# ralexstokes/ethereum_consensus

Measured on NVIDIA H100. Metric: fast_aggregate_verify tuples/s, higher is better.
Workload: dtype u32 limbs (381-bit Fp), u32 SHA-256 words

## Files before the change

ethereum_consensus_b200/csrc/groups.cuh:

```cuda
#pragma once
#include "curve.cuh"
#include "fpl.cuh"

namespace b200 {

enum : int32_t {
    BLS_SUCCESS = 0, BLS_BAD_ENCODING = 1, BLS_POINT_NOT_ON_CURVE = 2, BLS_POINT_NOT_IN_GROUP = 3,
    BLS_AGGR_TYPE_MISMATCH = 4, BLS_VERIFY_FAIL = 5, BLS_PK_IS_INFINITY = 6, BLS_BAD_SCALAR = 7
};

typedef Aff<Fp> G1Aff;
typedef Jac<Fp> G1Jac;
typedef Aff<Fp2> G2Aff;
typedef Jac<Fp2> G2Jac;

B200_HD bool fp_from_be48_masked(Fp& r, const uint8_t* b, bool mask_flags) {
    Fp raw;
    fp_from_be_bytes_raw(raw, b);
    if (mask_flags) raw.l[11] &= 0x1fffffffu;
    const Fp p = fp_p();
    if (fp_geq_raw(raw, p)) return false;
    fp_to_mont(r, raw);
    return true;
}
B200_HD bool bytes_all_zero(const uint8_t* b, int n) {
    uint32_t acc = 0;
    for (int i = 0; i < n; i++) acc |= b[i];
    return acc == 0;
}

B200_HD int32_t g1_uncompress(G1Aff& out, const uint8_t b[48]) {
    const uint8_t f = b[0];
    out.inf = 0;
    if (!(f & 0x80)) return BLS_BAD_ENCODING;
    if (f & 0x40) {
        if ((f & 0x3f) == 0 && bytes_all_zero(b + 1, 47)) { out.inf = 1; out.x = fp_zero(); out.y = fp_zero(); return BLS_SUCCESS; }
        return BLS_BAD_ENCODING;
    }
    Fp x, y2, y;
    if (!fp_from_be48_masked(x, b, true)) return BLS_BAD_ENCODING;
    fp_sqr(y2, x);
    fp_mul(y2, y2, x);
    const Fp four = B200_FP_B_G1;
    fp_add(y2, y2, four);
    if (!fp_sqrt(y, y2)) return BLS_POINT_NOT_ON_CURVE;
    if (fp_is_lex_largest(y) != ((f & 0x20) != 0)) fp_neg(y, y);
    out.x = x; out.y = y;
    return BLS_SUCCESS;
}

B200_HD bool g1_in_subgroup(const G1Aff& p) {
    if (p.inf) return true;
    G1Jac t, t2;
    jac_mul_u64(t, p.x, p.y, B200_Z_ABS);
    jac_mul_u64_jac(t2, t, B200_Z_ABS);
    const Fp beta = B200_FP_BETA;
    Fp bx, ny;
    fp_mul(bx, p.x, beta);
    fp_neg(ny, p.y);
    return jac_eq_aff(t2, bx, ny);
}

B200_HD int32_t g1_uncompress_lazy(G1Aff& out, const uint8_t b[48]) {
    const uint8_t f = b[0];
    out.inf = 0;
    if (!(f & 0x80)) return BLS_BAD_ENCODING;
    if (f & 0x40) {
        if ((f & 0x3f) == 0 && bytes_all_zero(b + 1, 47)) { out.inf = 1; out.x = fp_zero(); out.y = fp_zero(); return BLS_SUCCESS; }
        return BLS_BAD_ENCODING;
    }
    Fp x;
    if (!fp_from_be48_masked(x, b, true)) return BLS_BAD_ENCODING;
    FpL xl = fpl_from_fp(x), y2, yl, c;
    f_sqr(y2, xl);
    f_mul(y2, y2, xl);
    f_add(y2, y2, curve_b<FpL>());
    fpl_pow(yl, y2, B200_EXP_TABLE(exp_sqrt));
    f_sqr(c, yl);
    if (!f_eq(c, y2)) return BLS_POINT_NOT_ON_CURVE;
    Fp y = fpl_canon(yl);
    if (fp_is_lex_largest(y) != ((f & 0x20) != 0)) fp_neg(y, y);
    out.x = x; out.y = y;
    return BLS_SUCCESS;
}
B200_HD bool g1_in_subgroup_lazy(const G1Aff& p) {
    if (p.inf) return true;
    const FpL px = fpl_from_fp(p.x), py = fpl_from_fp(p.y);
    Jac<FpL> t, t2;
    jac_mul_u64(t, px, py, B200_Z_ABS);
    jac_mul_u64_jac(t2, t, B200_Z_ABS);
    const Fp beta = B200_FP_BETA;
    FpL bx, ny;
    f_mul(bx, px, fpl_from_fp(beta));
    f_neg(ny, py);
    return jac_eq_aff(t2, bx, ny);
}

B200_HD int32_t g1_key_validate(G1Aff& out, const uint8_t b[48]) {
#if defined(B200_G1_CANONICAL_FP)
    int32_t rc = g1_uncompress(out, b);
    if (rc) return rc;
    if (out.inf) return BLS_PK_IS_INFINITY;
    if (!g1_in_subgroup(out)) return BLS_POINT_NOT_IN_GROUP;
#else
    int32_t rc = g1_uncompress_lazy(out, b);
    if (rc) return rc;
    if (out.inf) return BLS_PK_IS_INFINITY;
    if (!g1_in_subgroup_lazy(out)) return BLS_POINT_NOT_IN_GROUP;
#endif
    return BLS_SUCCESS;
}

B200_HD void g1_compress(uint8_t out[48], const G1Aff& a) {
    if (a.inf) { for (int i = 0; i < 48; i++) out[i] = 0; out[0] = 0xc0; return; }
    Fp raw;
    fp_from_mont(raw, a.x);
    fp_to_be_bytes_raw(out, raw);
    out[0] |= 0x80;
    if (fp_is_lex_largest(a.y)) out[0] |= 0x20;
}

B200_BIG int32_t g2_uncompress(G2Aff& out, const uint8_t b[96]) {
    const uint8_t f = b[0];
    out.inf = 0;
    if (!(f & 0x80)) return BLS_BAD_ENCODING;
    if (f & 0x40) {
        if ((f & 0x3f) == 0 && bytes_all_zero(b + 1, 95)) { out.inf = 1; out.x = fp2_zero(); out.y = fp2_zero(); return BLS_SUCCESS; }
        return BLS_BAD_ENCODING;
    }
    Fp2 x, y2, y;
    if (!fp_from_be48_masked(x.c1, b, true)) return BLS_BAD_ENCODING;
    if (!fp_from_be48_masked(x.c0, b + 48, false)) return BLS_BAD_ENCODING;
    fp2_sqr(y2, x);
    fp2_mul(y2, y2, x);
    const Fp2 bb = B200_FP2_B_G2;
    fp2_add(y2, y2, bb);
    if (!fp2_sqrt(y, y2)) return BLS_POINT_NOT_ON_CURVE;
    if (fp2_is_lex_largest(y) != ((f & 0x20) != 0)) fp2_neg(y, y);
    out.x = x; out.y = y;
    return BLS_SUCCESS;
}

B200_HD void g2_compress(uint8_t out[96], const G2Aff& a) {
    if (a.inf) { for (int i = 0; i < 96; i++) out[i] = 0; out[0] = 0xc0; return; }
    Fp raw;
    fp_from_mont(raw, a.x.c1);
    fp_to_be_bytes_raw(out, raw);
    fp_from_mont(raw, a.x.c0);
// ... 52 lines not shown
```

ethereum_consensus_b200/build.py:

```python
from __future__ import annotations

import os
import subprocess
import sys
from concurrent.futures import ThreadPoolExecutor
from pathlib import Path

PKG = Path(__file__).resolve().parent
CSRC = PKG / "csrc"
LIB = PKG / "libb200_consensus.so"
OBJ = PKG / "build"
NVCC = os.environ.get("NVCC", "/usr/local/cuda/bin/nvcc")
ARCH = ["-gencode", "arch=compute_90a,code=sm_90a"]
FLAGS = [*ARCH, "-lineinfo", "-O3", "-std=c++17",
         "-Xcompiler", "-fPIC,-fvisibility=hidden", "--expt-relaxed-constexpr"]
DEFAULT_PTXAS_OPT = {"bls_g1.cu": 1, "bls_g2.cu": 1, "bls_vm.cu": 1}


def _stale(target: Path, deps) -> bool:
    if not target.exists():
        return True
    t = target.stat().st_mtime
    return any(Path(d).stat().st_mtime > t for d in deps)


def build(force: bool = False, verbose: bool = False, defines=(), suffix: str = "", ptxas_opt=None) -> Path:
    global LIB, OBJ
    env_opt = {kv.split(":")[0]: int(kv.split(":")[1]) for kv in os.environ.get("B200_PTXAS_OPT", "").split(",") if kv}
    ptxas_opt = {**DEFAULT_PTXAS_OPT, **env_opt, **dict(ptxas_opt or {})}
    if suffix:
        LIB = PKG / f"libb200_consensus{suffix}.so"
        OBJ = PKG / f"build{suffix}"
    srcs = sorted(CSRC.glob("*.cu"))
    hdrs = sorted(CSRC.glob("*.cuh")) + sorted(CSRC.glob("*.h")) + sorted((PKG.parent / "include").glob("*.h"))
    OBJ.mkdir(exist_ok=True)
    jobs = []
    def command(s, o):
        cmd = [NVCC, *FLAGS, *[f"-D{d}" for d in defines], "-c", str(s), "-o", str(o)]
        if s.name in ptxas_opt and int(ptxas_opt[s.name]) != 3:
            cmd[1:1] = ["-Xptxas", f"-O{int(ptxas_opt[s.name])}"]
        return cmd

    for s in srcs:
        o = OBJ / (s.stem + ".o")
        stamp = o.with_suffix(".cmd")
        if force or _stale(o, [s] + hdrs) or not stamp.exists() or stamp.read_text() != " ".join(command(s, o)):
            jobs.append((s, o))

    def cc(job):
        s, o = job
        cmd = command(s, o)
        stamp = o.with_suffix(".cmd")
        if verbose:
            cmd.insert(1, "-Xptxas=-v")
        r = subprocess.run(cmd, capture_output=True, text=True)
        if r.returncode != 0:
            raise RuntimeError(f"nvcc failed for {s.name}:\n{r.stdout}\n{r.stderr}")
        stamp.write_text(" ".join(command(s, o)))
        return r.stderr

    with ThreadPoolExecutor(max_workers=min(8, max(1, len(jobs)))) as ex:
        for msg in ex.map(cc, jobs):
            if verbose and msg:
                print(msg, file=sys.stderr)
    objs = [OBJ / (s.stem + ".o") for s in srcs]
    if force or jobs or _stale(LIB, objs):
        cmd = [NVCC, "-shared", "-o", str(LIB), *map(str, objs), *ARCH,
               "-Xcompiler", "-fPIC", "-cudart", "static"]
        r = subprocess.run(cmd, capture_output=True, text=True)
# ... 12 lines not shown
```

ethereum_consensus_b200/crypto.py:

```python
from __future__ import annotations

import ctypes as C
from typing import Sequence

import numpy as np

from . import _lib
from .ssz import hash

BLS_DST = b"BLS_SIG_BLS12381G2_XMD:SHA-256_SSWU_RO_POP_"
BLS_PUBLIC_KEY_BYTES_LEN = 48
BLS_SIGNATURE_BYTES_LEN = 96
INFINITY_COMPRESSED_SIGNATURE = bytes([0xC0]) + bytes(95)

_BLST_TEXT = {1: "bad encoding", 2: "point not on curve", 3: "point not in group", 4: "aggregation type mismatch",
              5: "verification failed", 6: "public key is infinity", 7: "bad scalar input"}

_lib.register_protos({
    "b200_verify_signature": (C.c_int32, [C.c_void_p, C.c_void_p, C.c_size_t, C.c_void_p]),
    "b200_fast_aggregate_verify": (C.c_int32, [C.c_void_p, C.c_size_t, C.c_void_p, C.c_size_t, C.c_void_p]),
    "b200_eth_fast_aggregate_verify": (C.c_int32, [C.c_void_p, C.c_size_t, C.c_void_p, C.c_size_t, C.c_void_p]),
    "b200_aggregate_verify": (C.c_int32, [C.c_void_p, C.c_size_t, C.c_void_p, C.c_void_p, C.c_size_t, C.c_void_p]),
    "b200_aggregate": (C.c_int32, [C.c_void_p, C.c_size_t, C.c_void_p]),
    "b200_eth_aggregate_public_keys": (C.c_int32, [C.c_void_p, C.c_size_t, C.c_void_p]),
# ... 173 lines not shown

    def __init__(self, pks_flat):
        n = (pks_flat.nbytes if hasattr(pks_flat, "nbytes") else len(pks_flat)) // 48
        _lib.check(_lib.lib().b200_registry_load(_lib.ptr(pks_flat), n), "registry_load")
        self.n = n

    def key_codes(self) -> np.ndarray:
        out = np.empty(max(self.n, 1), dtype=np.int32)
        _lib.check(_lib.lib().b200_registry_key_codes(_lib.ptr(out), self.n), "registry_key_codes")
        return out[:self.n]

    def verify_batch(self, indices, offsets, msgs32, sigs, extra_keys=None) -> np.ndarray:
        idx = np.ascontiguousarray(indices, dtype=np.uint32)
        off = np.ascontiguousarray(offsets, dtype=np.uint32)
        t = _batch_size(off, msgs32, sigs, indices=idx)
        out = np.empty(max(t, 1), dtype=np.int32)
        if extra_keys is not None and _nbytes(extra_keys):
            if _nbytes(extra_keys) % 48:
                raise ValueError("extra keys must be 48 bytes each")
            _lib.check(_lib.lib().b200_fast_aggregate_verify_batch_mixed(_lib.ptr(extra_keys), _nbytes(extra_keys) // 48, _lib.ptr(idx), _lib.ptr(off),
                                                                         _lib.ptr(msgs32), _lib.ptr(sigs), t, _lib.ptr(out)), "verify_batch_mixed")
        else:
            _lib.check(_lib.lib().b200_fast_aggregate_verify_batch_indexed(_lib.ptr(idx), _lib.ptr(off), _lib.ptr(msgs32),
                                                                           _lib.ptr(sigs), t, _lib.ptr(out)), "verify_batch_indexed")
        return out[:t]

    def verify_batch_all(self, indices, offsets, msgs32, sigs, seed: bytes = None) -> bool:
        idx = np.ascontiguousarray(indices, dtype=np.uint32)
        off = np.ascontiguousarray(offsets, dtype=np.uint32)
        t = _batch_size(off, msgs32, sigs, indices=idx, seed=seed)
        sd = np.frombuffer(bytes(seed), dtype=np.uint8) if seed is not None else None
        ok = C.c_int32(0)
        _lib.check(_lib.lib().b200_fast_aggregate_verify_batch_indexed_all(_lib.ptr(idx), _lib.ptr(off), _lib.ptr(msgs32), _lib.ptr(sigs), t,
                                                                           _lib.ptr(sd) if sd is not None else 0, C.byref(ok)), "verify_batch_indexed_all")
        return bool(ok.value)


def last_kernel_ms() -> float:
    return float(_lib.lib().b200_last_kernel_ms())


def last_dominant_kernel_ms() -> float:
    return float(_lib.lib().b200_last_dominant_kernel_ms())


def fp_selftest(n: int = 1 << 16, seed: int = 1) -> int:
    m = C.c_uint32(0)
    _lib.check(_lib.lib().b200_fp_selftest(n, seed, C.byref(m)), "fp_selftest")
    return int(m.value)


FP_EVAL_OPS = {"fp_mul": 0, "fp_sqr": 1, "fpl_mul": 2, "fpl_sqr": 3, "fp_add": 4, "fp_sub": 5, "fp_neg": 6, "fpl_add": 7,
               "fpl_sub": 8, "fpl_neg": 9, "fp_add_raw": 10, "fp_sub_raw": 11, "fp_inv_kaliski": 12, "fp_inv_fermat": 13,
               "fp_sqrt": 14, "fpl_pow_sqrt": 15, "fp_is_lex_largest": 16,
               "fp2_mul": 32, "fp2_sqr": 33, "fp2_inv": 34, "fp2_sqrt": 35, "fp2_sgn0": 36}


def fp_eval(op: str, a, b=None) -> np.ndarray:
    a = np.ascontiguousarray(a, dtype=np.uint32)
    b = np.zeros_like(a) if b is None else np.ascontiguousarray(b, dtype=np.uint32)
    if a.ndim != 2 or a.shape[1] != 24 or b.shape != a.shape:
        raise ValueError("operands must be uint32[n, 24]")
    out = np.zeros((max(a.shape[0], 1), 25), dtype=np.uint32)
    _lib.check(_lib.lib().b200_fp_eval(FP_EVAL_OPS[op], a.shape[0], _lib.ptr(a), _lib.ptr(b), _lib.ptr(out)), f"fp_eval({op})")
    return out[:a.shape[0]]


CURVE_EVAL_OPS = {"g1l_add_mixed": 0, "g1l_add": 1, "g1l_in_subgroup": 2,
                  "g2_add": 32, "g2_add_mixed": 33, "g2_double": 34, "g2_in_subgroup": 35, "g2_psi": 36,
                  "g2_clear_cofactor": 37, "g2_sswu_iso": 38, "g2_h2c_finish": 39}


def curve_eval(op: str, a, b=None) -> np.ndarray:
    a = np.ascontiguousarray(a, dtype=np.uint32)
    b = np.zeros_like(a) if b is None else np.ascontiguousarray(b, dtype=np.uint32)
    if a.ndim != 2 or a.shape[1] != 73 or b.shape != a.shape:
        raise ValueError("operands must be uint32[n, 73]")
    out = np.zeros((max(a.shape[0], 1), 73), dtype=np.uint32)
    _lib.check(_lib.lib().b200_curve_eval(CURVE_EVAL_OPS[op], a.shape[0], _lib.ptr(a), _lib.ptr(b), _lib.ptr(out)),
               f"curve_eval({op})")
    return out[:a.shape[0]]


def tune(knob: str, value: int) -> None:
    _lib.check(_lib.lib().b200_tune(knob.encode(), int(value)), f"tune({knob})")


def vm_load_programs(blob) -> None:
    a = np.ascontiguousarray(blob, dtype=np.uint32)
    _lib.check(_lib.lib().b200_vm_load_programs(_lib.ptr(a), a.size), "vm_load_programs")


def measure_int_peak(kind: int) -> float:
    g = C.c_double(0)
    _lib.check(_lib.lib().b200_measure_int_peak(kind, C.byref(g)), "measure_int_peak")
    return float(g.value)
```

ethereum_consensus_b200/csrc/bls_g1.cu:

```cuda
#if defined(B200_G1_SQR_VIA_MUL)
#define B200_FP_SQR_VIA_MUL 1
#endif
#if !defined(B200_G1_INLINE_MUL)
#define B200_FP_MUL_CALL 1
#endif
#define B200_POW_TAB_SMEM 1
#include <cuda_runtime.h>

#include "bls_kernels.cuh"

namespace b200 {
namespace {

__device__ __forceinline__ void g1_validate_body(const uint8_t* __restrict__ keys, uint32_t n, G1Aff* __restrict__ out,
                                                 int32_t* __restrict__ codes) {
    const uint32_t i = blockIdx.x * blockDim.x + threadIdx.x;
    if (i >= n) return;
    __align__(16) uint8_t b[48];
    const uint4* src = reinterpret_cast<const uint4*>(keys + size_t(i) * 48);
    uint4* dst = reinterpret_cast<uint4*>(b);
    dst[0] = src[0]; dst[1] = src[1]; dst[2] = src[2];
    G1Aff p;
    const int32_t rc = g1_key_validate(p, b);
    codes[i] = rc;
// ... 132 lines not shown
        const uint32_t bu = fp_sub_raw(u, x, y), bv = fp_sub_raw_portable(v, x, y);
        if (bu != bv || !fp_eq(u, v)) bad++;
        fp_add(u, x, y); fp_sub(u, u, y);
        if (!fp_eq(u, x)) bad++;
        fp_sub(u, x, y); fp_sub(v, y, x); fp_neg(v, v);
        if (!fp_eq(u, v)) bad++;
        fp_dbl(u, x); fp_add(v, x, x);
        if (!fp_eq(u, v)) bad++;
        fp_neg(u, x); fp_add(u, u, x);
        if (!fp_is_zero(u)) bad++;
        fp_add_masked_raw(u, x, y, 0u);
        if (!fp_eq(u, x)) bad++;
        fp_add_masked_raw(u, x, y, 0xffffffffu); fp_add_raw_portable(v, x, y);
        if (!fp_eq(u, v)) bad++;
    }
    if ((i & 63) == 0 && !fp_is_zero(a)) {
        fp_inv(t, a); fp_mul(t, t, a);
        if (!fp_eq(t, fp_one())) bad++;
        Fp k, f;
        fp_inv_kaliski(k, a); fp_inv_fermat(f, a);
        if (!fp_eq(k, f)) bad++;
        fp_inv_kaliski(k, fp_zero());
        if (!fp_is_zero(k)) bad++;
    }
    if (bad) atomicAdd(out_mismatch, bad);
}

__global__ void k_fp_eval(int32_t op, uint32_t n, const uint32_t* __restrict__ a, const uint32_t* __restrict__ b,
                          uint32_t* __restrict__ out) {
    const uint32_t i = blockIdx.x * blockDim.x + threadIdx.x;
    if (i >= n) return;
    Fp x, y, r = fp_zero();
    for (int k = 0; k < 12; k++) { x.l[k] = a[size_t(i) * kFpEvalIn + k]; y.l[k] = b[size_t(i) * kFpEvalIn + k]; }
    const FpL xl = fpl_from_fp(x), yl = fpl_from_fp(y);
    FpL rl;
    uint32_t flag = 0;
    switch (op) {
    case FP_EVAL_MUL: fp_mul(r, x, y); break;
    case FP_EVAL_SQR: fp_sqr(r, x); break;
    case FPL_EVAL_MUL: f_mul(rl, xl, yl); r = rl.v; break;
    case FPL_EVAL_SQR: f_sqr(rl, xl); r = rl.v; break;
    case FP_EVAL_ADD: fp_add(r, x, y); break;
    case FP_EVAL_SUB: fp_sub(r, x, y); break;
    case FP_EVAL_NEG: fp_neg(r, x); break;
    case FPL_EVAL_ADD: f_add(rl, xl, yl); r = rl.v; break;
    case FPL_EVAL_SUB: f_sub(rl, xl, yl); r = rl.v; break;
    case FPL_EVAL_NEG: f_neg(rl, xl); r = rl.v; break;
    case FP_EVAL_ADD_RAW: flag = fp_add_raw(r, x, y); break;
    case FP_EVAL_SUB_RAW: flag = fp_sub_raw(r, x, y); break;
    case FP_EVAL_INV_KALISKI: fp_inv_kaliski(r, x); break;
    case FP_EVAL_INV_FERMAT: fp_inv_fermat(r, x); break;
    case FP_EVAL_SQRT: flag = fp_sqrt(r, x) ? 1u : 0u; break;
    case FPL_EVAL_POW_SQRT: fpl_pow(rl, xl, B200_EXP_TABLE(exp_sqrt)); r = rl.v; break;
    case FP_EVAL_IS_LEX_LARGEST: flag = fp_is_lex_largest(x) ? 1u : 0u; break;
    default: break;
    }
    uint32_t* o = out + size_t(i) * kFpEvalOut;
    for (int k = 0; k < 12; k++) { o[k] = r.l[k]; o[12 + k] = 0; }
    o[24] = flag;
}

__global__ void k_curve_eval(int32_t op, uint32_t n, const uint32_t* __restrict__ a, const uint32_t* __restrict__ b,
                             uint32_t* __restrict__ out) {
    const uint32_t i = blockIdx.x * blockDim.x + threadIdx.x;
    if (i >= n) return;
    const uint32_t* pa = a + size_t(i) * kCurveEvalWords;
    const uint32_t* pb = b + size_t(i) * kCurveEvalWords;
    Jac<FpL> p, q, r;
    for (int k = 0; k < 12; k++) {
        p.x.v.l[k] = pa[k]; p.y.v.l[k] = pa[24 + k]; p.z.v.l[k] = pa[48 + k];
        q.x.v.l[k] = pb[k]; q.y.v.l[k] = pb[24 + k]; q.z.v.l[k] = pb[48 + k];
    }
    jac_set_inf(r);
    uint32_t flag = 0;
    switch (op) {
    case CURVE_G1L_ADD_MIXED: jac_add_mixed(r, p, q.x, q.y); break;
    case CURVE_G1L_ADD: jac_add(r, p, q); break;
    case CURVE_G1L_IN_SUBGROUP: {
        G1Aff s;
        s.x = p.x.v; s.y = p.y.v; s.inf = pa[72];
        flag = g1_in_subgroup_lazy(s) ? 1u : 0u;
        break;
    }
    default: break;
    }
    uint32_t* o = out + size_t(i) * kCurveEvalWords;
    for (int k = 0; k < 72; k++) o[k] = 0;
    for (int k = 0; k < 12; k++) { o[k] = r.x.v.l[k]; o[24 + k] = r.y.v.l[k]; o[48 + k] = r.z.v.l[k]; }
    o[72] = flag;
}

}

template <class K>
static size_t with_pow_tab(K kernel, unsigned threads) {
    const size_t bytes = fp_pow_smem_bytes(threads);
    static const void* seen[16];
    static size_t granted[16];
    static int n_seen = 0;
    const void* key = reinterpret_cast<const void*>(kernel);
    for (int i = 0; i < n_seen; i++)
        if (seen[i] == key) {
            if (granted[i] < bytes) { cudaFuncSetAttribute(kernel, cudaFuncAttributeMaxDynamicSharedMemorySize, int(bytes)); granted[i] = bytes; }
            return bytes;
        }
    cudaFuncSetAttribute(kernel, cudaFuncAttributeMaxDynamicSharedMemorySize, int(bytes));
    if (n_seen < 16) { seen[n_seen] = key; granted[n_seen++] = bytes; }
    return bytes;
}
static int g_g1_variant = 7;
static uint32_t g_g1_small_n = 3u * 148u * 384u;
void set_g1_small_n(uint32_t n) { g_g1_small_n = n; }
void set_g1_variant(int v) { if (v >= 0 && v <= 7) g_g1_variant = v; }
void launch_g1_validate(const uint8_t* keys, uint32_t n, G1Aff* out, int32_t* codes, void* stream, int cta) {
    if (!n) return;
    cudaStream_t st = static_cast<cudaStream_t>(stream);
    switch (g_g1_variant) {
    case 6: k_g1_validate_r128<<<(n + 511) / 512, 512, with_pow_tab(k_g1_validate_r128, 512), st>>>(keys, n, out, codes); break;
    case 0: k_g1_validate_main<<<(n + 255) / 256, 256, with_pow_tab(k_g1_validate_main, 256), st>>>(keys, n, out, codes); break;
    default:
        if (cta == 128 || (cta != 384 && n <= g_g1_small_n))
            k_g1_validate_r168<<<(n + 127) / 128, 128, with_pow_tab(k_g1_validate_r168, 128), st>>>(keys, n, out, codes);
        else
            k_g1_validate_r168<<<(n + 383) / 384, 384, with_pow_tab(k_g1_validate_r168, 384), st>>>(keys, n, out, codes);
        break;
    }
}
void launch_g1_aggregate(const G1Aff* keys, const int32_t* key_codes, const uint32_t* index, const uint32_t* off,
                         uint32_t n_tuples, G1Aff* agg, G1Pre* agg_pre, int32_t* pk_code, uint32_t* flags,
                         uint32_t extra_flags, void* stream, G1Jac* agg_jac) {
    if (!n_tuples) return;
    k_g1_aggregate<<<(n_tuples + kAggWarps - 1) / kAggWarps, 32 * kAggWarps, with_pow_tab(k_g1_aggregate, 32 * kAggWarps),
                     static_cast<cudaStream_t>(stream)>>>(
        keys, key_codes, index, off, n_tuples, agg, agg_pre, pk_code, flags, extra_flags, agg_jac);
}
void launch_g1_compress(const G1Aff* p, uint8_t* out48, void* stream) {
    k_g1_compress<<<1, 32, with_pow_tab(k_g1_compress, 32), static_cast<cudaStream_t>(stream)>>>(p, out48);
}
void launch_neg_g1(G1Aff* out, G1Pre* out_pre, void* stream) { k_neg_g1<<<1, 32, 0, static_cast<cudaStream_t>(stream)>>>(out, out_pre); }
void launch_fp_selftest(uint32_t n, uint32_t seed, uint32_t* out_mismatch, void* stream) {
    k_fp_selftest<<<(n + 127) / 128, 128, with_pow_tab(k_fp_selftest, 128), static_cast<cudaStream_t>(stream)>>>(n, seed, out_mismatch);
}
void launch_fp_eval(int32_t op, uint32_t n, const uint32_t* a, const uint32_t* b, uint32_t* out, void* stream) {
    if (!n) return;
    k_fp_eval<<<(n + 127) / 128, 128, with_pow_tab(k_fp_eval, 128), static_cast<cudaStream_t>(stream)>>>(op, n, a, b, out);
}
void launch_curve_eval(int32_t op, uint32_t n, const uint32_t* a, const uint32_t* b, uint32_t* out, void* stream) {
    if (!n) return;
    k_curve_eval<<<(n + 127) / 128, 128, with_pow_tab(k_curve_eval, 128), static_cast<cudaStream_t>(stream)>>>(op, n, a, b, out);
}

}
```

ethereum_consensus_b200/csrc/bls_kernels.cuh:

```cuda
#pragma once
#include <cstddef>
#include <cstdint>

#include "groups.cuh"
#include "fp12.cuh"

namespace b200 {

struct G1Pre {
    Fp xz, y, z3;
    uint32_t inf;
};

enum : uint32_t { TUPLE_FLAG_EMPTY = 1u, TUPLE_FLAG_AGG_INF = 2u };
enum : int32_t { SIG_OK = 0, SIG_NOT_IN_GROUP = -1 };

void set_g1_variant(int v);
void set_g1_small_n(uint32_t n);
void set_small_cta(int threads);
void set_vm_team16_max(uint32_t n);
void set_vm_cta(int threads);
void launch_g1_validate(const uint8_t* keys, uint32_t n, G1Aff* out, int32_t* codes, void* stream, int cta = 0);
void launch_g1_aggregate(const G1Aff* keys, const int32_t* key_codes, const uint32_t* index, const uint32_t* off,
                         uint32_t n_tuples, G1Aff* agg, G1Pre* agg_pre, int32_t* pk_code, uint32_t* flags,
                         uint32_t extra_flags, void* stream, G1Jac* agg_jac = nullptr);
void launch_rlc_scale(const G1Jac* agg, const G2Aff* sig, const int32_t* pk_code, const uint32_t* flags, const int32_t* sig_code,
                      const uint32_t* seed_words, uint64_t t0, uint32_t n, G1Pre* out_g1, G2Jac* out_g2, int32_t* bad, void* stream);
uint32_t launch_rlc_reduce(const Fp12* f_in, const G2Jac* q_in, uint32_t n, Fp12* f_out, G2Jac* q_out, void* stream);
void launch_rlc_finish(const G2Jac* q, G2Aff* out, void* stream);
void launch_fp12_one(Fp12* out, void* stream);
void launch_g2_sig_decode(const uint8_t* sigs, uint32_t n, G2Aff* out, int32_t* sig_code, void* stream);
void launch_hash_to_g2(const uint8_t* msgs, const uint32_t* moff, uint32_t n, G2Aff* out, void* tmp_jac, void* stream);
void launch_miller(const G1Aff* g1, const uint32_t* g1_idx, const G2Aff* g2, const uint32_t* g2_idx,
                   const uint32_t* pair_tuple, const int32_t* pk_code, const uint32_t* flags, const int32_t* sig_code,
                   uint32_t n_pairs, Fp12* f, void* stream);
void launch_final(const Fp12* f, const uint32_t* pair_off, const int32_t* pk_code, const uint32_t* flags,
                  const int32_t* sig_code, uint32_t n_tuples, int32_t* out_codes, void* stream);
int vm_init(void* stream);
int vm_load_programs(const uint32_t* blob, size_t n_words, void* stream);
void launch_vm_miller(const G1Pre* g1, const uint32_t* g1_idx, const G2Aff* g2, const uint32_t* g2_idx,
                      const uint32_t* pair_tuple, const int32_t* pk_code, const uint32_t* flags, const int32_t* sig_code,
                      uint32_t n_pairs, Fp12* f, void* stream);
void launch_vm_final(const Fp12* f, const uint32_t* pair_off, const int32_t* pk_code, const uint32_t* flags,
                     const int32_t* sig_code, uint32_t n_tuples, int32_t* out_codes, void* stream);
void launch_g2_sum_compress(const G2Aff* sigs, const int32_t* sig_code, uint32_t n, uint8_t* out96, int32_t* out_code, void* stream);
void launch_g1_compress(const G1Aff* p, uint8_t* out48, void* stream);
void launch_neg_g1(G1Aff* out, G1Pre* out_pre, void* stream);
void launch_fp_selftest(uint32_t n, uint32_t seed, uint32_t* out_mismatch, void* stream);
enum : int32_t {
    FP_EVAL_MUL = 0, FP_EVAL_SQR = 1, FPL_EVAL_MUL = 2, FPL_EVAL_SQR = 3,
    FP_EVAL_ADD = 4, FP_EVAL_SUB = 5, FP_EVAL_NEG = 6, FPL_EVAL_ADD = 7, FPL_EVAL_SUB = 8, FPL_EVAL_NEG = 9,
    FP_EVAL_ADD_RAW = 10, FP_EVAL_SUB_RAW = 11, FP_EVAL_INV_KALISKI = 12, FP_EVAL_INV_FERMAT = 13,
    FP_EVAL_SQRT = 14, FPL_EVAL_POW_SQRT = 15, FP_EVAL_IS_LEX_LARGEST = 16,
    FP_EVAL_N_OPS = 17,
    FP2_EVAL_MUL = 32, FP2_EVAL_SQR = 33, FP2_EVAL_INV = 34, FP2_EVAL_SQRT = 35, FP2_EVAL_SGN0 = 36,
    FP2_EVAL_END = 37
};
constexpr uint32_t kFpEvalIn = 24, kFpEvalOut = 25;
void launch_fp_eval(int32_t op, uint32_t n, const uint32_t* a, const uint32_t* b, uint32_t* out, void* stream);
void launch_fp2_eval(int32_t op, uint32_t n, const uint32_t* a, const uint32_t* b, uint32_t* out, void* stream);
enum : int32_t {
    CURVE_G1L_ADD_MIXED = 0, CURVE_G1L_ADD = 1, CURVE_G1L_IN_SUBGROUP = 2,
    CURVE_G1_N_OPS = 3,
    CURVE_G2_ADD = 32, CURVE_G2_ADD_MIXED = 33, CURVE_G2_DOUBLE = 34, CURVE_G2_IN_SUBGROUP = 35, CURVE_G2_PSI = 36,
    CURVE_G2_CLEAR_COFACTOR = 37, CURVE_G2_SSWU_ISO = 38, CURVE_G2_H2C_FINISH = 39,
    CURVE_G2_END = 40
};
constexpr uint32_t kCurveEvalWords = 73;
void launch_curve_eval(int32_t op, uint32_t n, const uint32_t* a, const uint32_t* b, uint32_t* out, void* stream);
void launch_curve2_eval(int32_t op, uint32_t n, const uint32_t* a, const uint32_t* b, uint32_t* out, void* stream);

}
```

ethereum_consensus_b200/csrc/capi_bls.cu:

```cuda
#include <algorithm>
#include <cctype>
#include <cstdlib>
#include <cstring>
#include <memory>
#include <random>
#include <string>
#include <vector>

#include "bls_kernels.cuh"
#include "comm.h"
#include "engine.h"

namespace b200 {

struct BlsState {
    cudaStream_t sb = nullptr, sc = nullptr;
    static constexpr uint32_t kMaxChunks = 16;
    cudaStream_t sd = nullptr, se = nullptr;
    cudaEvent_t ev_ck[kMaxChunks] = {nullptr}, ev_join = nullptr;
    uint32_t chunks = 1, chunk_min_tuples = 2048;
    int chunk_k1_cta = 128;
    bool chunk_alt = true;
    bool key_split = true;
    int k1_first_cta = 128;
// ... 570 lines not shown
    int32_t rc = check_ready(e);
    if (rc) return rc;
    BlsState* s;
    rc = bls_state(e, &s);
    if (rc) return rc;
    if (!knob) return B200_ERR_BAD_ARG;
    for (const Knob& k : kKnobs)
        if (strcmp(k.name, knob) == 0) { k.set(*s, value); return B200_SUCCESS; }
    return B200_ERR_BAD_ARG;
}

int32_t b200_vm_load_programs(const uint32_t* blob, size_t n_words) {
    Engine& e = engine();
    Guard g(e);
    int32_t rc = check_ready(e);
    if (rc) return rc;
    BlsState* s;
    rc = bls_state(e, &s);
    if (rc) return rc;
    B200_CUDA_TRY(cudaStreamSynchronize(e.stream));
    if (vm_load_programs(blob, n_words, e.stream) != 0) { e.last_error = "malformed pairing-VM program blob"; return B200_ERR_BAD_ARG; }
    return B200_SUCCESS;
}

float b200_last_dominant_kernel_ms(void) {
    Engine& e = engine();
    return e.bls ? static_cast<BlsState*>(e.bls)->last_dominant_ms : 0.f;
}

int32_t b200_fp_selftest(uint32_t n, uint32_t seed, uint32_t* mismatches) {
    Engine& e = engine();
    Guard g(e);
    int32_t rc = check_ready(e);
    if (rc) return rc;
    if (!mismatches) return B200_ERR_BAD_ARG;
    uint32_t* d = nullptr;
    B200_CUDA_TRY(cudaMalloc(&d, 4));
    B200_CUDA_TRY(cudaMemsetAsync(d, 0, 4, e.stream));
    launch_fp_selftest(n, seed, d, e.stream);
    e.launches++;
    B200_CUDA_TRY(cudaGetLastError());
    B200_CUDA_TRY(cudaMemcpyAsync(mismatches, d, 4, cudaMemcpyDeviceToHost, e.stream));
    B200_CUDA_TRY(cudaStreamSynchronize(e.stream));
    cudaFree(d);
    return B200_SUCCESS;
}

int32_t b200_fp_eval(int32_t op, uint32_t n, const uint32_t* a, const uint32_t* b, uint32_t* out) {
    Engine& e = engine();
    Guard g(e);
    int32_t rc = check_ready(e);
    if (rc) return rc;
    const bool fp2 = op >= FP2_EVAL_MUL && op < FP2_EVAL_END;
    if (!(fp2 || (op >= 0 && op < FP_EVAL_N_OPS)) || n > (1u << 24)) return B200_ERR_BAD_ARG;
    if (n == 0) return B200_SUCCESS;
    if (!a || !b || !out) return B200_ERR_BAD_ARG;
    const size_t in_bytes = size_t(n) * kFpEvalIn * 4, out_bytes = size_t(n) * kFpEvalOut * 4;
    uint32_t* d = nullptr;
    B200_CUDA_TRY(cudaMalloc(&d, 2 * in_bytes + out_bytes));
    uint32_t* da = d;
    uint32_t* db = d + size_t(n) * kFpEvalIn;
    uint32_t* dout = db + size_t(n) * kFpEvalIn;
    cudaMemcpyAsync(da, a, in_bytes, cudaMemcpyHostToDevice, e.stream);
    cudaMemcpyAsync(db, b, in_bytes, cudaMemcpyHostToDevice, e.stream);
    if (fp2) launch_fp2_eval(op, n, da, db, dout, e.stream);
    else launch_fp_eval(op, n, da, db, dout, e.stream);
    e.launches++;
    cudaError_t ce = cudaGetLastError();
    if (ce == cudaSuccess) ce = cudaMemcpyAsync(out, dout, out_bytes, cudaMemcpyDeviceToHost, e.stream);
    if (ce == cudaSuccess) ce = cudaStreamSynchronize(e.stream);
    cudaFree(d);
    if (ce != cudaSuccess) { e.last_error = cudaGetErrorString(ce); return B200_ERR_CUDA; }
    return B200_SUCCESS;
}

int32_t b200_curve_eval(int32_t op, uint32_t n, const uint32_t* a, const uint32_t* b, uint32_t* out) {
    Engine& e = engine();
    Guard g(e);
    int32_t rc = check_ready(e);
    if (rc) return rc;
    const bool g2 = op >= CURVE_G2_ADD && op < CURVE_G2_END;
    if (!(g2 || (op >= 0 && op < CURVE_G1_N_OPS)) || n > (1u << 24)) return B200_ERR_BAD_ARG;
    if (n == 0) return B200_SUCCESS;
    if (!a || !b || !out) return B200_ERR_BAD_ARG;
    const size_t bytes = size_t(n) * kCurveEvalWords * 4;
    uint32_t* d = nullptr;
    B200_CUDA_TRY(cudaMalloc(&d, 3 * bytes));
    uint32_t* da = d;
    uint32_t* db = d + size_t(n) * kCurveEvalWords;
    uint32_t* dout = db + size_t(n) * kCurveEvalWords;
    cudaMemcpyAsync(da, a, bytes, cudaMemcpyHostToDevice, e.stream);
    cudaMemcpyAsync(db, b, bytes, cudaMemcpyHostToDevice, e.stream);
    if (g2) launch_curve2_eval(op, n, da, db, dout, e.stream);
    else launch_curve_eval(op, n, da, db, dout, e.stream);
    e.launches++;
    cudaError_t ce = cudaGetLastError();
    if (ce == cudaSuccess) ce = cudaMemcpyAsync(out, dout, bytes, cudaMemcpyDeviceToHost, e.stream);
    if (ce == cudaSuccess) ce = cudaStreamSynchronize(e.stream);
    cudaFree(d);
    if (ce != cudaSuccess) { e.last_error = cudaGetErrorString(ce); return B200_ERR_CUDA; }
    return B200_SUCCESS;
}

int32_t b200_fast_aggregate_verify_batch(const uint8_t* pks_flat, const uint32_t* pk_offsets, const uint8_t* msgs32,
                                         const uint8_t* sigs, size_t n_tuples, int32_t* out_codes) {
    Engine& e = engine();
    Guard g(e);
// ... 337 lines not shown
```

ethereum_consensus_b200/csrc/curve.cuh:

```cuda
#pragma once
#include "fp2.cuh"

namespace b200 {

B200_HD void f_add(Fp& r, const Fp& a, const Fp& b) { fp_add(r, a, b); }
B200_HD void f_sub(Fp& r, const Fp& a, const Fp& b) { fp_sub(r, a, b); }
B200_HD void f_mul(Fp& r, const Fp& a, const Fp& b) { fp_mul(r, a, b); }
B200_HD void f_sqr(Fp& r, const Fp& a) { fp_sqr(r, a); }
B200_HD void f_neg(Fp& r, const Fp& a) { fp_neg(r, a); }
B200_HD void f_dbl(Fp& r, const Fp& a) { fp_dbl(r, a); }
B200_HD void f_inv(Fp& r, const Fp& a) { fp_inv(r, a); }
B200_HD bool f_is_zero(const Fp& a) { return fp_is_zero(a); }
B200_HD bool f_eq(const Fp& a, const Fp& b) { return fp_eq(a, b); }
B200_HD void f_add(Fp2& r, const Fp2& a, const Fp2& b) { fp2_add(r, a, b); }
B200_HD void f_sub(Fp2& r, const Fp2& a, const Fp2& b) { fp2_sub(r, a, b); }
B200_HD void f_mul(Fp2& r, const Fp2& a, const Fp2& b) { fp2_mul(r, a, b); }
B200_HD void f_sqr(Fp2& r, const Fp2& a) { fp2_sqr(r, a); }
B200_HD void f_neg(Fp2& r, const Fp2& a) { fp2_neg(r, a); }
B200_HD void f_dbl(Fp2& r, const Fp2& a) { fp2_dbl(r, a); }
B200_HD void f_inv(Fp2& r, const Fp2& a) { fp2_inv(r, a); }
B200_HD bool f_is_zero(const Fp2& a) { return fp2_is_zero(a); }
B200_HD bool f_eq(const Fp2& a, const Fp2& b) { return fp2_eq(a, b); }
template <class F> B200_HD F f_one();
template <> B200_HD Fp f_one<Fp>() { return fp_one(); }
// ... 41 lines not shown
    f_add(t, p.x, B);
    f_sqr(t, t);
    f_sub(t, t, A);
    f_sub(t, t, C);
    f_dbl(D, t);
    f_dbl(E, A);
    f_add(E, E, A);
    f_sqr(Fq, E);
    F z3;
    f_mul(z3, p.y, p.z);
    f_dbl(z3, z3);
    F x3;
    f_dbl(t, D);
    f_sub(x3, Fq, t);
    f_sub(t, D, x3);
    f_mul(t, E, t);
    f_dbl(C, C); f_dbl(C, C); f_dbl(C, C);
    f_sub(r.y, t, C);
    r.x = x3;
    r.z = z3;
}

template <class F> B200_BIG void jac_add_mixed(Jac<F>& r, const Jac<F>& p, const F& qx, const F& qy) {
    if (jac_is_inf(p)) { r.x = qx; r.y = qy; r.z = f_one<F>(); return; }
    F zz, zzz, u2, s2, h, rr;
    f_sqr(zz, p.z);
    f_mul(zzz, zz, p.z);
    f_mul(u2, qx, zz);
    f_mul(s2, qy, zzz);
    f_sub(h, u2, p.x);
    f_sub(rr, s2, p.y);
    if (f_is_zero(h)) {
        if (f_is_zero(rr)) { Jac<F> t; t.x = qx; t.y = qy; t.z = f_one<F>(); jac_double(r, t); }
        else jac_set_inf(r);
        return;
    }
    F hh, hhh, v, x3, t;
    f_sqr(hh, h);
    f_mul(hhh, hh, h);
    f_mul(v, p.x, hh);
    f_sqr(x3, rr);
    f_sub(x3, x3, hhh);
    f_dbl(t, v);
    f_sub(x3, x3, t);
    f_sub(t, v, x3);
    f_mul(t, rr, t);
    F y1h;
    f_mul(y1h, p.y, hhh);
    f_sub(r.y, t, y1h);
    f_mul(r.z, p.z, h);
    r.x = x3;
}

template <class F> B200_BIG void jac_add(Jac<F>& r, const Jac<F>& p, const Jac<F>& q) {
    if (jac_is_inf(p)) { r = q; return; }
    if (jac_is_inf(q)) { r = p; return; }
    F z1z1, z2z2, u1, u2, s1, s2, h, rr, t;
    f_sqr(z1z1, p.z);
    f_sqr(z2z2, q.z);
    f_mul(u1, p.x, z2z2);
    f_mul(u2, q.x, z1z1);
    f_mul(t, q.z, z2z2);
    f_mul(s1, p.y, t);
    f_mul(t, p.z, z1z1);
    f_mul(s2, q.y, t);
    f_sub(h, u2, u1);
    f_sub(rr, s2, s1);
    if (f_is_zero(h)) {
        if (f_is_zero(rr)) jac_double(r, p); else jac_set_inf(r);
        return;
    }
    F hh, hhh, v, x3;
    f_sqr(hh, h);
    f_mul(hhh, hh, h);
    f_mul(v, u1, hh);
    f_sqr(x3, rr);
    f_sub(x3, x3, hhh);
    f_dbl(t, v);
    f_sub(x3, x3, t);
    f_sub(t, v, x3);
    f_mul(t, rr, t);
    f_mul(s1, s1, hhh);
    f_sub(r.y, t, s1);
    f_mul(t, p.z, q.z);
    f_mul(r.z, t, h);
    r.x = x3;
}

template <class F> B200_BIG void jac_to_aff(Aff<F>& a, const Jac<F>& p) {
    if (jac_is_inf(p)) { a.inf = 1; a.x = f_zero<F>(); a.y = f_zero<F>(); return; }
    F zi, zi2, zi3;
    f_inv(zi, p.z);
    f_sqr(zi2, zi);
    f_mul(zi3, zi2, zi);
    f_mul(a.x, p.x, zi2);
    f_mul(a.y, p.y, zi3);
    a.inf = 0;
}

template <class F> B200_HD bool jac_eq_aff(const Jac<F>& p, const F& qx, const F& qy) {
    if (jac_is_inf(p)) return false;
    F zz, zzz, a, b;
    f_sqr(zz, p.z);
    f_mul(zzz, zz, p.z);
    f_mul(a, qx, zz);
    f_mul(b, qy, zzz);
    return f_eq(a, p.x) && f_eq(b, p.y);
}

template <class F> B200_BIG void jac_mul_u64(Jac<F>& r, const F& qx, const F& qy, uint64_t k) {
    Jac<F> acc;
    jac_set_inf(acc);
    bool started = false;
#pragma unroll 1
    for (int bit = 63; bit >= 0; bit--) {
        if (started) jac_double(acc, acc);
        if ((k >> bit) & 1) {
            jac_add_mixed(acc, acc, qx, qy);
            started = true;
        }
    }
    r = acc;
}
template <class F> B200_BIG void jac_mul_u64_jac(Jac<F>& r, const Jac<F>& q, uint64_t k) {
    Jac<F> acc;
    jac_set_inf(acc);
    bool started = false;
#pragma unroll 1
    for (int bit = 63; bit >= 0; bit--) {
        if (started) jac_double(acc, acc);
        if ((k >> bit) & 1) {
            jac_add(acc, acc, q);
            started = true;
        }
    }
    r = acc;
}

}
```

ethereum_consensus_b200/csrc/fpl.cuh:

```cuda
#pragma once
#include "curve.cuh"

namespace b200 {

struct FpL {
    Fp v;
};

B200_HD Fp fp_2p() { Fp r = B200_FP_2P; return r; }

B200_HD void fpl_reduce_2p(Fp& r) {
    const Fp pp = fp_2p();
    Fp t;
    const uint32_t borrow = fp_sub_raw(t, r, pp);
    fp_select(r, t, borrow == 0);
}
B200_HD FpL fpl_from_fp(const Fp& a) { FpL r; r.v = a; return r; }
B200_HD Fp fpl_canon(const FpL& a) { Fp r = a.v; fp_reduce_once(r); return r; }

B200_HD void f_add(FpL& r, const FpL& a, const FpL& b) {
    fp_add_raw(r.v, a.v, b.v);
    fpl_reduce_2p(r.v);
}
B200_HD void f_sub(FpL& r, const FpL& a, const FpL& b) {
// ... 45 lines not shown
#else
    fp_sqr_emul_core(out.l, a.v.l);
#endif
#endif
    r.v = out;
}
B200_HD bool f_is_zero(const FpL& a) { return fp_is_zero(fpl_canon(a)); }
B200_HD bool f_eq(const FpL& a, const FpL& b) { return fp_eq(fpl_canon(a), fpl_canon(b)); }
template <> B200_HD FpL f_one<FpL>() { return fpl_from_fp(fp_one()); }
template <> B200_HD FpL f_zero<FpL>() { return fpl_from_fp(fp_zero()); }
template <> B200_HD FpL curve_b<FpL>() { Fp b = B200_FP_B_G1; return fpl_from_fp(b); }

B200_BIG void fpl_pow(FpL& r, const FpL& a, const uint32_t* e) {
    PowTab tab;
    tab.set(0, a.v);
    {
        FpL a2, cur = a;
        f_sqr(a2, a);
#pragma unroll 1
        for (int k = 1; k < kPowTabEntries; k++) { f_mul(cur, cur, a2); tab.set(k, cur.v); }
    }
    int i = 383;
    while (i >= 0 && !((e[i >> 5] >> (i & 31)) & 1u)) i--;
    if (i < 0) { r = f_one<FpL>(); return; }
    FpL acc, t;
    bool started = false;
#pragma unroll 1
    while (i >= 0) {
        if (!((e[i >> 5] >> (i & 31)) & 1u)) {
            f_sqr(acc, acc);
            i--;
            continue;
        }
        int l = i + 1 < 4 ? i + 1 : 4;
        const int lo = i - l + 1;
        uint64_t two = e[lo >> 5];
        if ((lo >> 5) + 1 < 12) two |= uint64_t(e[(lo >> 5) + 1]) << 32;
        uint32_t w = uint32_t(two >> (lo & 31)) & ((1u << l) - 1u);
        while (!(w & 1u)) { w >>= 1; l--; }
        if (started) {
#pragma unroll 1
            for (int k = 0; k < l; k++) f_sqr(acc, acc);
            tab.get(t.v, int(w >> 1));
            f_mul(acc, acc, t);
        } else {
            tab.get(acc.v, int(w >> 1));
            started = true;
        }
        i -= l;
    }
    r = acc;
}

}
```

Measured before the change: 32290.

## Rework G1 subgroup check with table-backed mixed-add scalar multiplication

Replaces the two generic jac_mul_u64 calls in the lazy G1 subgroup check with a custom double-and-add that reads its base point from a PowTab (likely shared or local memory) and uses mixed additions. The second multiplication is done in an affine-equivalent frame: the intermediate Jacobian point is used as the affine base, and the comparison target is rescaled by Z^2 and Z^3. This keeps fewer live registers and makes the second scalar multiply use cheaper mixed additions. It adds an early infinity check and depends on PowTab accessor costs and on the scaled-comparison maths being correct.

```diff
diff --git a/ethereum_consensus_b200/csrc/groups.cuh b/ethereum_consensus_b200/csrc/groups.cuh
--- a/ethereum_consensus_b200/csrc/groups.cuh
+++ b/ethereum_consensus_b200/csrc/groups.cuh
@@ -83,17 +83,49 @@
     out.x = x; out.y = y;
     return BLS_SUCCESS;
 }
+B200_HD void g1l_mul_zabs(Jac<FpL>& r, const PowTab& tab, int slot) {
+    Jac<FpL> acc;
+    jac_set_inf(acc);
+    bool started = false;
+#pragma unroll 1
+    for (int bit = 63; bit >= 0; bit--) {
+        if (started) jac_double(acc, acc);
+        if ((B200_Z_ABS >> bit) & 1) {
+            FpL qx, qy;
+            tab.get(qx.v, slot);
+            tab.get(qy.v, slot + 1);
+            jac_add_mixed(acc, acc, qx, qy);
+            started = true;
+        }
+    }
+    r = acc;
+}
 B200_HD bool g1_in_subgroup_lazy(const G1Aff& p) {
     if (p.inf) return true;
-    const FpL px = fpl_from_fp(p.x), py = fpl_from_fp(p.y);
-    Jac<FpL> t, t2;
-    jac_mul_u64(t, px, py, B200_Z_ABS);
-    jac_mul_u64_jac(t2, t, B200_Z_ABS);
+    PowTab tab;
+    tab.set(0, p.x);
+    tab.set(1, p.y);
+    Jac<FpL> t;
+    g1l_mul_zabs(t, tab, 0);
+    if (jac_is_inf(t)) return false;
     const Fp beta = B200_FP_BETA;
-    FpL bx, ny;
+    FpL zz, bx, ny, px, py;
+    tab.get(px.v, 0);
+    tab.get(py.v, 1);
+    f_sqr(zz, t.z);
     f_mul(bx, px, fpl_from_fp(beta));
+    f_mul(bx, bx, zz);
+    f_mul(zz, zz, t.z);
     f_neg(ny, py);
-    return jac_eq_aff(t2, bx, ny);
+    f_mul(ny, ny, zz);
+    tab.set(0, t.x.v);
+    tab.set(1, t.y.v);
+    tab.set(2, bx.v);
+    tab.set(3, ny.v);
+    g1l_mul_zabs(t, tab, 0);
+    tab.get(bx.v, 2);
+    tab.get(ny.v, 3);
+    return jac_eq_aff(t, bx, ny);
 }
 
 B200_HD int32_t g1_key_validate(G1Aff& out, const uint8_t b[48]) {
```

After: 32600 (median of 6 runs). Within noise of the previous version (+1.0%).

## Use fixed addition chain for G1 sqrt and cache Z powers in subgroup check

Applied to the files above, without the earlier changes.

Replaces the table-driven windowed exponentiation in lazy G1 decompression with a hard-coded addition chain for the square-root exponent, which removes table lookups and shared-memory use. The second scalar multiplication in the G1 subgroup check now precomputes Z^2 and Z^3 of the fixed addend once, saving two multiplications per add. The G1 validate kernels no longer reserve the power table in shared memory and set the preferred carveout to zero, and the ptxas optimisation level for bls_g1.cu goes from 1 to 2. Together these trade code size and register pressure for fewer field multiplications.

```diff
diff --git a/ethereum_consensus_b200/build.py b/ethereum_consensus_b200/build.py
--- a/ethereum_consensus_b200/build.py
+++ b/ethereum_consensus_b200/build.py
@@ -14,7 +14,7 @@
 ARCH = ["-gencode", "arch=compute_90a,code=sm_90a"]
 FLAGS = [*ARCH, "-lineinfo", "-O3", "-std=c++17",
          "-Xcompiler", "-fPIC,-fvisibility=hidden", "--expt-relaxed-constexpr"]
-DEFAULT_PTXAS_OPT = {"bls_g1.cu": 1, "bls_g2.cu": 1, "bls_vm.cu": 1}
+DEFAULT_PTXAS_OPT = {"bls_g1.cu": 2, "bls_g2.cu": 1, "bls_vm.cu": 1}
 
 
 def _stale(target: Path, deps) -> bool:
diff --git a/ethereum_consensus_b200/crypto.py b/ethereum_consensus_b200/crypto.py
--- a/ethereum_consensus_b200/crypto.py
+++ b/ethereum_consensus_b200/crypto.py
@@ -249,7 +249,7 @@
 
 FP_EVAL_OPS = {"fp_mul": 0, "fp_sqr": 1, "fpl_mul": 2, "fpl_sqr": 3, "fp_add": 4, "fp_sub": 5, "fp_neg": 6, "fpl_add": 7,
                "fpl_sub": 8, "fpl_neg": 9, "fp_add_raw": 10, "fp_sub_raw": 11, "fp_inv_kaliski": 12, "fp_inv_fermat": 13,
-               "fp_sqrt": 14, "fpl_pow_sqrt": 15, "fp_is_lex_largest": 16,
+               "fp_sqrt": 14, "fpl_pow_sqrt": 15, "fp_is_lex_largest": 16, "fpl_sqrt_chain": 18,
                "fp2_mul": 32, "fp2_sqr": 33, "fp2_inv": 34, "fp2_sqrt": 35, "fp2_sgn0": 36}
 
 
diff --git a/ethereum_consensus_b200/csrc/bls_g1.cu b/ethereum_consensus_b200/csrc/bls_g1.cu
--- a/ethereum_consensus_b200/csrc/bls_g1.cu
+++ b/ethereum_consensus_b200/csrc/bls_g1.cu
@@ -208,6 +208,7 @@
     case FP_EVAL_INV_FERMAT: fp_inv_fermat(r, x); break;
     case FP_EVAL_SQRT: flag = fp_sqrt(r, x) ? 1u : 0u; break;
     case FPL_EVAL_POW_SQRT: fpl_pow(rl, xl, B200_EXP_TABLE(exp_sqrt)); r = rl.v; break;
+    case FPL_EVAL_SQRT_CHAIN: fpl_sqrt_chain(rl, xl); r = rl.v; break;
     case FP_EVAL_IS_LEX_LARGEST: flag = fp_is_lex_largest(x) ? 1u : 0u; break;
     default: break;
     }
@@ -264,6 +265,22 @@
     if (n_seen < 16) { seen[n_seen] = key; granted[n_seen++] = bytes; }
     return bytes;
 }
+template <class K>
+static size_t k1_smem(K kernel, unsigned threads) {
+#if defined(B200_G1_CANONICAL_FP)
+    return with_pow_tab(kernel, threads);
+#else
+    (void)threads;
+    static const void* done[3];
+    static int n_done = 0;
+    const void* key = reinterpret_cast<const void*>(kernel);
+    for (int i = 0; i < n_done; i++)
+        if (done[i] == key) return 0;
+    cudaFuncSetAttribute(kernel, cudaFuncAttributePreferredSharedMemoryCarveout, 0);
+    if (n_done < 3) done[n_done++] = key;
+    return 0;
+#endif
+}
 static int g_g1_variant = 7;
 static uint32_t g_g1_small_n = 3u * 148u * 384u;
 void set_g1_small_n(uint32_t n) { g_g1_small_n = n; }
@@ -272,13 +289,13 @@
     if (!n) return;
     cudaStream_t st = static_cast<cudaStream_t>(stream);
     switch (g_g1_variant) {
-    case 6: k_g1_validate_r128<<<(n + 511) / 512, 512, with_pow_tab(k_g1_validate_r128, 512), st>>>(keys, n, out, codes); break;
-    case 0: k_g1_validate_main<<<(n + 255) / 256, 256, with_pow_tab(k_g1_validate_main, 256), st>>>(keys, n, out, codes); break;
+    case 6: k_g1_validate_r128<<<(n + 511) / 512, 512, k1_smem(k_g1_validate_r128, 512), st>>>(keys, n, out, codes); break;
+    case 0: k_g1_validate_main<<<(n + 255) / 256, 256, k1_smem(k_g1_validate_main, 256), st>>>(keys, n, out, codes); break;
     default:
         if (cta == 128 || (cta != 384 && n <= g_g1_small_n))
-            k_g1_validate_r168<<<(n + 127) / 128, 128, with_pow_tab(k_g1_validate_r168, 128), st>>>(keys, n, out, codes);
+            k_g1_validate_r168<<<(n + 127) / 128, 128, k1_smem(k_g1_validate_r168, 128), st>>>(keys, n, out, codes);
         else
-            k_g1_validate_r168<<<(n + 383) / 384, 384, with_pow_tab(k_g1_validate_r168, 384), st>>>(keys, n, out, codes);
+            k_g1_validate_r168<<<(n + 383) / 384, 384, k1_smem(k_g1_validate_r168, 384), st>>>(keys, n, out, codes);
         break;
     }
 }
diff --git a/ethereum_consensus_b200/csrc/bls_kernels.cuh b/ethereum_consensus_b200/csrc/bls_kernels.cuh
--- a/ethereum_consensus_b200/csrc/bls_kernels.cuh
+++ b/ethereum_consensus_b200/csrc/bls_kernels.cuh
@@ -53,6 +53,7 @@
     FP_EVAL_ADD_RAW = 10, FP_EVAL_SUB_RAW = 11, FP_EVAL_INV_KALISKI = 12, FP_EVAL_INV_FERMAT = 13,
     FP_EVAL_SQRT = 14, FPL_EVAL_POW_SQRT = 15, FP_EVAL_IS_LEX_LARGEST = 16,
     FP_EVAL_N_OPS = 17,
+    FPL_EVAL_SQRT_CHAIN = 18,
     FP2_EVAL_MUL = 32, FP2_EVAL_SQR = 33, FP2_EVAL_INV = 34, FP2_EVAL_SQRT = 35, FP2_EVAL_SGN0 = 36,
     FP2_EVAL_END = 37
 };
diff --git a/ethereum_consensus_b200/csrc/capi_bls.cu b/ethereum_consensus_b200/csrc/capi_bls.cu
--- a/ethereum_consensus_b200/csrc/capi_bls.cu
+++ b/ethereum_consensus_b200/csrc/capi_bls.cu
@@ -646,7 +646,7 @@
     int32_t rc = check_ready(e);
     if (rc) return rc;
     const bool fp2 = op >= FP2_EVAL_MUL && op < FP2_EVAL_END;
-    if (!(fp2 || (op >= 0 && op < FP_EVAL_N_OPS)) || n > (1u << 24)) return B200_ERR_BAD_ARG;
+    if (!(fp2 || (op >= 0 && op < FP_EVAL_N_OPS) || op == FPL_EVAL_SQRT_CHAIN) || n > (1u << 24)) return B200_ERR_BAD_ARG;
     if (n == 0) return B200_SUCCESS;
     if (!a || !b || !out) return B200_ERR_BAD_ARG;
     const size_t in_bytes = size_t(n) * kFpEvalIn * 4, out_bytes = size_t(n) * kFpEvalOut * 4;
diff --git a/ethereum_consensus_b200/csrc/curve.cuh b/ethereum_consensus_b200/csrc/curve.cuh
--- a/ethereum_consensus_b200/csrc/curve.cuh
+++ b/ethereum_consensus_b200/csrc/curve.cuh
@@ -117,16 +117,14 @@
     r.x = x3;
 }
 
-template <class F> B200_BIG void jac_add(Jac<F>& r, const Jac<F>& p, const Jac<F>& q) {
+template <class F> B200_HD void jac_add_zz(Jac<F>& r, const Jac<F>& p, const Jac<F>& q, const F& z2z2, const F& z2z3) {
     if (jac_is_inf(p)) { r = q; return; }
     if (jac_is_inf(q)) { r = p; return; }
-    F z1z1, z2z2, u1, u2, s1, s2, h, rr, t;
+    F z1z1, u1, u2, s1, s2, h, rr, t;
     f_sqr(z1z1, p.z);
-    f_sqr(z2z2, q.z);
     f_mul(u1, p.x, z2z2);
     f_mul(u2, q.x, z1z1);
-    f_mul(t, q.z, z2z2);
-    f_mul(s1, p.y, t);
+    f_mul(s1, p.y, z2z3);
     f_mul(t, p.z, z1z1);
     f_mul(s2, q.y, t);
     f_sub(h, u2, u1);
@@ -151,6 +149,14 @@
     f_mul(r.z, t, h);
     r.x = x3;
 }
+template <class F> B200_BIG void jac_add(Jac<F>& r, const Jac<F>& p, const Jac<F>& q) {
+    if (jac_is_inf(p)) { r = q; return; }
+    if (jac_is_inf(q)) { r = p; return; }
+    F z2z2, z2z3;
+    f_sqr(z2z2, q.z);
+    f_mul(z2z3, q.z, z2z2);
+    jac_add_zz(r, p, q, z2z2, z2z3);
+}
 
 template <class F> B200_BIG void jac_to_aff(Aff<F>& a, const Jac<F>& p) {
     if (jac_is_inf(p)) { a.inf = 1; a.x = f_zero<F>(); a.y = f_zero<F>(); return; }
@@ -201,5 +207,22 @@
     }
     r = acc;
 }
-
-}
+template <class F> B200_BIG void jac_mul_u64_jac_cached(Jac<F>& r, const Jac<F>& q, uint64_t k) {
+    F zz, zzz;
+    f_sqr(zz, q.z);
+    f_mul(zzz, q.z, zz);
+    Jac<F> acc;
+    jac_set_inf(acc);
+    bool started = false;
+#pragma unroll 1
+    for (int bit = 63; bit >= 0; bit--) {
+        if (started) jac_double(acc, acc);
+        if ((k >> bit) & 1) {
+            jac_add_zz(acc, acc, q, zz, zzz);
+            started = true;
+        }
+    }
+    r = acc;
+}
+
+}
diff --git a/ethereum_consensus_b200/csrc/fpl.cuh b/ethereum_consensus_b200/csrc/fpl.cuh
--- a/ethereum_consensus_b200/csrc/fpl.cuh
+++ b/ethereum_consensus_b200/csrc/fpl.cuh
@@ -121,4 +121,11 @@
     r = acc;
 }
 
+B200_HD void fpl_sqr_n(FpL& a, int n) {
+#pragma unroll 1
+    for (int k = 0; k < n; k++) f_sqr(a, a);
 }
+
+}
+
+#include "fpl_sqrt_chain.cuh"
diff --git a/ethereum_consensus_b200/csrc/fpl_sqrt_chain.cuh b/ethereum_consensus_b200/csrc/fpl_sqrt_chain.cuh
--- /dev/null
+++ b/ethereum_consensus_b200/csrc/fpl_sqrt_chain.cuh
@@ -0,0 +1,153 @@
+#pragma once
+
+namespace b200 {
+
+B200_BIG void fpl_sqrt_chain(FpL& r, const FpL& x1) {
+    FpL x2, x3, x5, x7, x9, x11, x13, x15, x21, x255, acc;
+    f_sqr(x2, x1);
+    f_mul(x3, x2, x1);
+    f_mul(x5, x3, x2);
+    f_mul(x7, x5, x2);
+    f_mul(x9, x7, x2);
+    f_mul(x11, x9, x2);
+    f_mul(x13, x11, x2);
+    f_mul(x15, x13, x2);
+    x21 = x3;
+    fpl_sqr_n(x21, 1);
+    f_mul(x21, x21, x15);
+    x255 = x15;
+    fpl_sqr_n(x255, 4);
+    f_mul(x255, x255, x15);
+    acc = x13;
+    fpl_sqr_n(acc, 9);
+    f_mul(acc, acc, x1);
+    fpl_sqr_n(acc, 4);
+    f_mul(acc, acc, x1);
+    fpl_sqr_n(acc, 7);
+    f_mul(acc, acc, x15);
+    fpl_sqr_n(acc, 4);
+    f_mul(acc, acc, x5);
+    fpl_sqr_n(acc, 6);
+    f_mul(acc, acc, x7);
+    fpl_sqr_n(acc, 6);
+    f_mul(acc, acc, x11);
+    fpl_sqr_n(acc, 8);
+    f_mul(acc, acc, x255);
+    fpl_sqr_n(acc, 6);
+    f_mul(acc, acc, x13);
+    fpl_sqr_n(acc, 6);
+    f_mul(acc, acc, x13);
+    fpl_sqr_n(acc, 6);
+    f_mul(acc, acc, x9);
+    fpl_sqr_n(acc, 3);
+    f_mul(acc, acc, x3);
+    fpl_sqr_n(acc, 7);
+    f_mul(acc, acc, x13);
+    fpl_sqr_n(acc, 4);
+    f_mul(acc, acc, x13);
+    fpl_sqr_n(acc, 6);
+    f_mul(acc, acc, x15);
+    fpl_sqr_n(acc, 5);
+    f_mul(acc, acc, x13);
+    fpl_sqr_n(acc, 4);
+    f_mul(acc, acc, x9);
+    fpl_sqr_n(acc, 8);
+    f_mul(acc, acc, x13);
+    fpl_sqr_n(acc, 6);
+    f_mul(acc, acc, x11);
+    fpl_sqr_n(acc, 5);
+    f_mul(acc, acc, x21);
+    fpl_sqr_n(acc, 4);
+    f_mul(acc, acc, x9);
+    fpl_sqr_n(acc, 5);
+    f_mul(acc, acc, x21);
+    fpl_sqr_n(acc, 4);
+    f_mul(acc, acc, x13);
+    fpl_sqr_n(acc, 4);
+    f_mul(acc, acc, x9);
+    fpl_sqr_n(acc, 6);
+    f_mul(acc, acc, x7);
+    fpl_sqr_n(acc, 4);
+    f_mul(acc, acc, x7);
+    fpl_sqr_n(acc, 5);
+    f_mul(acc, acc, x9);
+    fpl_sqr_n(acc, 4);
+    f_mul(acc, acc, x7);
+    fpl_sqr_n(acc, 8);
+    f_mul(acc, acc, x9);
+    fpl_sqr_n(acc, 3);
+    f_mul(acc, acc, x7);
+    fpl_sqr_n(acc, 5);
+    f_mul(acc, acc, x7);
+    fpl_sqr_n(acc, 7);
+    f_mul(acc, acc, x5);
+    fpl_sqr_n(acc, 7);
+    f_mul(acc, acc, x9);
+    fpl_sqr_n(acc, 5);
+    f_mul(acc, acc, x11);
+    fpl_sqr_n(acc, 4);
+    f_mul(acc, acc, x15);
+    fpl_sqr_n(acc, 3);
+    f_mul(acc, acc, x3);
+    fpl_sqr_n(acc, 5);
+    f_mul(acc, acc, x7);
+    fpl_sqr_n(acc, 4);
+    f_mul(acc, acc, x3);
+    fpl_sqr_n(acc, 8);
+    f_mul(acc, acc, x13);
+    fpl_sqr_n(acc, 7);
+    f_mul(acc, acc, x21);
+    fpl_sqr_n(acc, 9);
+    f_mul(acc, acc, x15);
+    fpl_sqr_n(acc, 5);
+    f_mul(acc, acc, x13);
+    fpl_sqr_n(acc, 3);
+    f_mul(acc, acc, x3);
+    fpl_sqr_n(acc, 8);
+    f_mul(acc, acc, x15);
+    fpl_sqr_n(acc, 3);
+    f_mul(acc, acc, x3);
+    fpl_sqr_n(acc, 7);
+    f_mul(acc, acc, x9);
+    fpl_sqr_n(acc, 9);
+    f_mul(acc, acc, x15);
+    fpl_sqr_n(acc, 6);
+    f_mul(acc, acc, x21);
+    fpl_sqr_n(acc, 9);
+    f_mul(acc, acc, x255);
+    fpl_sqr_n(acc, 8);
+    f_mul(acc, acc, x255);
+    fpl_sqr_n(acc, 5);
+    f_mul(acc, acc, x21);
+    fpl_sqr_n(acc, 1);
+    f_mul(acc, acc, x1);
+    fpl_sqr_n(acc, 8);
+    f_mul(acc, acc, x21);
+    fpl_sqr_n(acc, 10);
+    f_mul(acc, acc, x255);
+    fpl_sqr_n(acc, 8);
+    f_mul(acc, acc, x255);
+    fpl_sqr_n(acc, 3);
+    f_mul(acc, acc, x7);
+    fpl_sqr_n(acc, 4);
+    f_mul(acc, acc, x7);
+    fpl_sqr_n(acc, 10);
+    f_mul(acc, acc, x255);
+    fpl_sqr_n(acc, 9);
+    f_mul(acc, acc, x255);
+    fpl_sqr_n(acc, 8);
+    f_mul(acc, acc, x255);
+    fpl_sqr_n(acc, 8);
+    f_mul(acc, acc, x255);
+    fpl_sqr_n(acc, 8);
+    f_mul(acc, acc, x255);
+    fpl_sqr_n(acc, 5);
+    f_mul(acc, acc, x21);
+    fpl_sqr_n(acc, 6);
+    f_mul(acc, acc, x21);
+    fpl_sqr_n(acc, 3);
+    f_mul(acc, acc, x3);
+    r = acc;
+}
+
+}
diff --git a/ethereum_consensus_b200/csrc/groups.cuh b/ethereum_consensus_b200/csrc/groups.cuh
--- a/ethereum_consensus_b200/csrc/groups.cuh
+++ b/ethereum_consensus_b200/csrc/groups.cuh
@@ -75,7 +75,7 @@
     f_sqr(y2, xl);
     f_mul(y2, y2, xl);
     f_add(y2, y2, curve_b<FpL>());
-    fpl_pow(yl, y2, B200_EXP_TABLE(exp_sqrt));
+    fpl_sqrt_chain(yl, y2);
     f_sqr(c, yl);
     if (!f_eq(c, y2)) return BLS_POINT_NOT_ON_CURVE;
     Fp y = fpl_canon(yl);
@@ -88,7 +88,7 @@
     const FpL px = fpl_from_fp(p.x), py = fpl_from_fp(p.y);
     Jac<FpL> t, t2;
     jac_mul_u64(t, px, py, B200_Z_ABS);
-    jac_mul_u64_jac(t2, t, B200_Z_ABS);
+    jac_mul_u64_jac_cached(t2, t, B200_Z_ABS);
     const Fp beta = B200_FP_BETA;
     FpL bx, ny;
     f_mul(bx, px, fpl_from_fp(beta));
```

Result: faster. 32090 before, 33220 after, median of 6 (+3.5%).
